# ImIntheMiddle/EmLoco

Measured on AMD Instinct MI355X. Metric: env-steps/sec (SMPL humanoid, num_envs), higher is better.
Workload: dtype f32

## Files before the change

### emloco_amd/csrc/emloco_types.h

```cpp
#pragma once
#define EMLOCO_PART_WORDS 800
#include "../../include/emloco_sim.h"
#define EMLOCO_PART_TAG(seq, part) ((seq) * 4u + (unsigned)(part))
#define EMLOCO_ERR_PART_TIMEOUT 1u

#define EMLOCO_TOPO_PARENT 0
#define EMLOCO_TOPO_DEPTH 24
#define EMLOCO_TOPO_CHILD 48
#define EMLOCO_TOPO_PDPACK 120
#define EMLOCO_TOPO_CAND 144
#define EMLOCO_TOPO_SCPAIR 240
#define EMLOCO_TOPO_WORDS 560

#define EMLOCO_MB_DYN 0
#define EMLOCO_MB_GEO 384
#define EMLOCO_MB_CAP 576
#define EMLOCO_MB_DRV 832
#define EMLOCO_MODEL_WORDS 1112

struct EmlocoSimDev {
    int n_env, n_cand, max_depth, sc_n;
    int sc_nseg;
    const int *topo;
    const float *model;
// ... 1 lines not shown
    const float *pd_target;
    float *rb_state, *contact_force, *dof_force, *lambda_ws;
    float sc_k, sc_c, sc_max_pen, sc_mu;
    const short *hf;
    int hf_nx, hf_ny;
    float hf_hs, hf_inv_hs, hf_vs, hf_ox, hf_oy, hf_pad_;
    const unsigned char *hf_mv;
    long long *prof;
    const long long *step_skip;
    const int *step_ids;
    int n_slots;
    const int *step_order;
    unsigned *step_ticks;
    int n_parts; unsigned part_seq;
    float *part_state;
    unsigned *part_flag;
    unsigned *err;
    int part_spin_max;
    int part_poison;
    unsigned long long *step_start;
    const unsigned *plan;
    int plan_n;
};
```

### emloco_amd/csrc/sim_capi.hip

```cpp
#include <hip/hip_runtime.h>
#include <cstdlib>
#include <cstdio>
#include <cstring>
#include <string>
#include <vector>
#ifdef EMLOCO_SIM_PAIR
#include "sim_pair_kernels.hip"
#define EMLOCO_SIM_ENVS_PER_WG 2
#else
#include "sim_kernels.hip"
#define EMLOCO_SIM_ENVS_PER_WG 1
#endif
#include "topology.h"
#include "model_pack.h"
#include "sim_state.h"
#include "sim_plan.h"
#include "capi_error.h"

using emloco::capi_fail;

namespace {

int check_device_error(EmlocoSim *s, const char *where) {
    if (!s->h_err) return EMLOCO_OK;
// ... 24 lines not shown

int emloco_sim_create(const EmlocoSimParams *params, int device, EmlocoSim **out) {
    if (!params || !out) return capi_fail(EMLOCO_E_ARG, "emloco_sim_create: null argument");
    if (params->n_sub < 1 || params->h <= 0.0f || params->n_iter < 0 || params->drive_mode < 0 || params->drive_mode > 1)
        return capi_fail(EMLOCO_E_ARG, "emloco_sim_create: n_sub >= 1, h > 0, n_iter >= 0, drive_mode 0 | 1 required");
    int n = 0;
    if (hipGetDeviceCount(&n) != hipSuccess || n == 0) return capi_fail(EMLOCO_E_NODEV, "no HIP device visible");
    if (device < 0 || device >= n) return capi_fail(EMLOCO_E_ARG, "emloco_sim_create: device index out of range");
    EMLOCO_HIPCHK(hipSetDevice(device));
    EmlocoSim *s = new EmlocoSim();
    s->device = device;
    s->prm = *params;
    *out = s;
    return EMLOCO_OK;
}

int emloco_sim_destroy(EmlocoSim *s) {
    if (!s) return EMLOCO_OK;
    (void)hipSetDevice(s->device);
    s->d_topo.release(); s->d_model.release();
    s->d_root.release(); s->d_dof.release(); s->d_tgt.release(); s->d_rb.release();
    s->d_cf.release(); s->d_df.release(); s->d_lws.release();
    s->d_ticks.release(); s->d_order.release(); s->d_order_ws.release();
    s->d_part_state.release(); s->d_part_flag.release(); s->d_plan.release();
    if (s->h_err) (void)hipHostFree(s->h_err);
    for (auto e : s->ev0) (void)hipEventDestroy(e);
    for (auto e : s->ev1) (void)hipEventDestroy(e);
    delete s;
    return EMLOCO_OK;
}

int emloco_sim_set_models(EmlocoSim *s, const EmlocoModelDesc *m) {
    if (!s || !m) return capi_fail(EMLOCO_E_ARG, "emloco_sim_set_models: null argument");
    if (s->prepared) return capi_fail(EMLOCO_E_STATE, "emloco_sim_set_models: sim already prepared");
    if (m->n_env < 1) return capi_fail(EMLOCO_E_ARG, "emloco_sim_set_models: n_env < 1");
    if (!s->topo.build(m->parent, m->geom_type))
        return capi_fail(EMLOCO_E_ARG, "emloco_sim_set_models: body tree must be depth-first, depth <= 8, <= 3 children, <= 96 contact candidates");
    const size_t E = (size_t)m->n_env, NBs = EMLOCO_NB, ND = EMLOCO_NDOF;
    s->n_env = m->n_env;
    s->h_off.assign(m->joint_off, m->joint_off + E * NBs * 3);
    s->h_mass.assign(m->mass, m->mass + E * NBs);
    s->h_com.assign(m->com, m->com + E * NBs * 3);
    s->h_inertia.assign(m->inertia, m->inertia + E * NBs * 6);
    s->h_ga.assign(m->geom_a, m->geom_a + E * NBs * 3);
    s->h_gb.assign(m->geom_b, m->geom_b + E * NBs * 3);
    s->h_gr.assign(m->geom_r, m->geom_r + E * NBs);
    s->h_kp.assign(m->kp, m->kp + E * ND);
// ... 159 lines not shown
int emloco_sim_tensor(EmlocoSim *s, int kind, void **dev_ptr, int64_t shape[2]) {
    if (!s || !dev_ptr || !shape) return capi_fail(EMLOCO_E_ARG, "emloco_sim_tensor: null argument");
    if (!s->prepared) return capi_fail(EMLOCO_E_STATE, "emloco_sim_tensor: call emloco_sim_prepare first");
    const int64_t E = s->n_env;
    switch (kind) {
        case EMLOCO_T_ROOT_STATE: *dev_ptr = s->d_root.p; shape[0] = E; shape[1] = 13; break;
        case EMLOCO_T_DOF_STATE: *dev_ptr = s->d_dof.p; shape[0] = E * EMLOCO_NDOF; shape[1] = 2; break;
        case EMLOCO_T_RIGID_BODY: *dev_ptr = s->d_rb.p; shape[0] = E * EMLOCO_NB; shape[1] = 13; break;
        case EMLOCO_T_CONTACT_FORCE: *dev_ptr = s->d_cf.p; shape[0] = E * EMLOCO_NB; shape[1] = 3; break;
        case EMLOCO_T_DOF_FORCE: *dev_ptr = s->d_df.p; shape[0] = E * EMLOCO_NDOF; shape[1] = 1; break;
        case EMLOCO_T_PD_TARGET: *dev_ptr = s->d_tgt.p; shape[0] = E; shape[1] = EMLOCO_NDOF; break;
        case EMLOCO_T_WARM_START: *dev_ptr = s->d_lws.p; shape[0] = E; shape[1] = EMLOCO_MAXCAND * 3; break;
        default: return capi_fail(EMLOCO_E_ARG, "emloco_sim_tensor: unknown tensor kind");
    }
    return EMLOCO_OK;
}

int emloco_sim_set_pd_targets(EmlocoSim *s, const float *dev_targets, void *stream) {
    if (!s || !dev_targets) return capi_fail(EMLOCO_E_ARG, "emloco_sim_set_pd_targets: null argument");
    if (!s->prepared) return capi_fail(EMLOCO_E_STATE, "emloco_sim_set_pd_targets: sim not prepared");
    if (dev_targets != s->d_tgt.p)
        EMLOCO_HIPCHK(hipMemcpyAsync(s->d_tgt.p, dev_targets, (size_t)s->n_env * EMLOCO_NDOF * 4, hipMemcpyDeviceToDevice, (hipStream_t)stream));
    s->prm.drive_mode = 0;
    return EMLOCO_OK;
}

int emloco_sim_set_dof_actuation_force(EmlocoSim *s, const float *dev_forces, void *stream) {
    if (!s || !dev_forces) return capi_fail(EMLOCO_E_ARG, "emloco_sim_set_dof_actuation_force: null argument");
    if (!s->prepared) return capi_fail(EMLOCO_E_STATE, "emloco_sim_set_dof_actuation_force: sim not prepared");
    if (dev_forces != s->d_tgt.p)
        EMLOCO_HIPCHK(hipMemcpyAsync(s->d_tgt.p, dev_forces, (size_t)s->n_env * EMLOCO_NDOF * 4, hipMemcpyDeviceToDevice, (hipStream_t)stream));
    s->prm.drive_mode = 1;
    return EMLOCO_OK;
}

static int launch_order(EmlocoSim *s, hipStream_t st) {
    if (s->order_ready) { s->order_ready = false; return EMLOCO_OK; }
    hipLaunchKernelGGL(emloco::sim_order_kernel, dim3(1), dim3(1024), 0, st, s->d_ticks.p, s->n_env, s->d_order.p, s->d_order_ws.p);
    EMLOCO_HIPCHK(hipGetLastError());
    return EMLOCO_OK;
}

static bool use_plan(const EmlocoSim *s, int n_sub) { return s->plan_n > 0 && s->plan_n_sub == n_sub; }

static int launch_step(EmlocoSim *s, int n_calls, EmlocoSimDev d, int n_slots, bool list, hipStream_t st) {
    EmlocoSimParams p = s->prm;
    p.n_sub = s->prm.n_sub * n_calls;
    const int slot = s->ev_head;
    const bool timed = s->timing && !list && (s->launch_no++ % s->timing_stride) == 0;
    if (timed) EMLOCO_HIPCHK(hipEventRecord(s->ev0[slot], st));
    d.n_parts = list ? 1 : (s->n_parts < p.n_sub ? s->n_parts : p.n_sub);
    d.part_seq = ++s->part_seq; d.part_state = s->d_part_state.p; d.part_flag = s->d_part_flag.p;
    d.part_spin_max = s->part_spin_max; d.part_poison = s->part_poison;
    d.n_slots = n_slots;
    unsigned grid = (unsigned)(((n_slots + EMLOCO_SIM_ENVS_PER_WG - 1) / EMLOCO_SIM_ENVS_PER_WG) * d.n_parts);
    if (!list && use_plan(s, p.n_sub)) { d.plan = s->d_plan.p; d.plan_n = s->plan_n; grid = (unsigned)s->plan_n; }
    if (d.hf) hipLaunchKernelGGL(emloco::sim_step_kernel<1>, dim3(grid), dim3(64), (size_t)s->lds_pad, st, p, d);
    else hipLaunchKernelGGL(emloco::sim_step_kernel<0>, dim3(grid), dim3(64), (size_t)s->lds_pad, st, p, d);
    EMLOCO_HIPCHK(hipGetLastError());
    if (timed) {
        EMLOCO_HIPCHK(hipEventRecord(s->ev1[slot], st));
        s->ev_head = (slot + 1) % EmlocoSim::kRing;
        if (s->ev_count < EmlocoSim::kRing) ++s->ev_count;
    }
    return EMLOCO_OK;
}

int emloco_sim_step(EmlocoSim *s, int n_calls, void *stream) {
    if (!s) return capi_fail(EMLOCO_E_ARG, "emloco_sim_step: null sim");
    if (!s->prepared) return capi_fail(EMLOCO_E_STATE, "emloco_sim_step: sim not prepared");
    if (n_calls < 1) return capi_fail(EMLOCO_E_ARG, "emloco_sim_step: n_calls < 1");
    if (const int rc = check_device_error(s, "emloco_sim_step")) return rc;
    hipStream_t st = (hipStream_t)stream;
    EmlocoSimDev d = s->dev;
    if (s->cost_order) {
        const int rc = launch_order(s, st);
        if (rc != EMLOCO_OK) return rc;
        d.step_order = s->d_order.p;
        d.step_ticks = s->d_ticks.p;
    }
    return launch_step(s, n_calls, d, s->n_env, false, st);
}

int emloco_sim_step_subset(EmlocoSim *s, int n_calls, const int64_t *dev_skip, const int32_t *dev_ids, int n_ids, void *stream) {
    if (!s) return capi_fail(EMLOCO_E_ARG, "emloco_sim_step_subset: null sim");
    if (!s->prepared) return capi_fail(EMLOCO_E_STATE, "emloco_sim_step_subset: sim not prepared");
    if (n_calls < 1) return capi_fail(EMLOCO_E_ARG, "emloco_sim_step_subset: n_calls < 1");
    if ((dev_skip == nullptr) == (dev_ids == nullptr)) return capi_fail(EMLOCO_E_ARG, "emloco_sim_step_subset: exactly one of skip flags / id list");
    if (dev_ids && (n_ids < 0 || n_ids > s->n_env)) return capi_fail(EMLOCO_E_ARG, "emloco_sim_step_subset: bad id count");
    if (dev_ids && n_ids == 0) return EMLOCO_OK;
    if (const int rc = check_device_error(s, "emloco_sim_step_subset")) return rc;
    EmlocoSimDev d = s->dev;
    d.step_skip = (const long long *)dev_skip;
    d.step_ids = (const int *)dev_ids;
    hipStream_t st = (hipStream_t)stream;
    if (s->cost_order) {
        d.step_ticks = s->d_ticks.p;
        if (dev_skip) {
            const int rc = launch_order(s, st);
            if (rc != EMLOCO_OK) return rc;
            d.step_order = s->d_order.p;
        }
    }
    return launch_step(s, n_calls, d, dev_ids ? n_ids : s->n_env, dev_ids != nullptr, st);
}

int emloco_sim_set_split(EmlocoSim *s, int n_parts) {
    if (!s) return capi_fail(EMLOCO_E_ARG, "emloco_sim_set_split: null sim");
    if (!s->prepared) return capi_fail(EMLOCO_E_STATE, "emloco_sim_set_split: sim not prepared");
    if (n_parts < 1 || n_parts > 4) return capi_fail(EMLOCO_E_ARG, "emloco_sim_set_split: 1 to 4 parts");
    if (n_parts > 1 && !s->d_part_state.p) {
        EMLOCO_HIPCHK(hipSetDevice(s->device));
// ... 176 lines not shown
```

### emloco_amd/csrc/sim_kernels.hip

```cpp
#include <hip/hip_runtime.h>
#include "dev_math.h"
#include "sim_math.h"
#define cross3 fcross3
#define dot3 fdot3
#define dot6 fdot6
#define qmul fqmul
#define qnormalize fqnormalize
#define q2mat fq2mat
#define matvec3 fmatvec3
#define rotvec2quat frotvec2quat
#define quat2rotvec fquat2rotvec
#include "emloco_types.h"
#include "fk_device.h"
#include "order_device.h"
#include "sim_plan.h"

namespace emloco {

#define NB EMLOCO_NB
#define NDOF EMLOCO_NDOF
#define MAXC EMLOCO_MAXC
#define MAXR (3 * EMLOCO_MAXC)
#define MAXCAND EMLOCO_MAXCAND
#define EMLOCO_WH_MAX 1.0f
#define YLEN 30

__device__ __forceinline__ constexpr int sidx(int a, int b) {
    return a <= b ? (a * (13 - a)) / 2 + (b - a) : (b * (13 - b)) / 2 + (a - b);
}

__device__ __forceinline__ int tri_index(int a, int b) {
    const int hi = a > b ? a : b, lo = a > b ? b : a;
    return ((hi * (hi + 1)) >> 1) + lo;
}

struct ContactMatrixSquare { static constexpr bool square = true; };
struct ContactMatrixPacked { static constexpr bool square = false; };
template <bool SQ>
// ... 187 lines not shown
                const float dv[3] = {0.0f - q[0], 0.0f - q[1], 0.0f - q[2]};
                const float side = dot3f(dv, fn);
                const float ifn = 1.0f / sqrtf(fn2);
                if (dsel >= 0.0f) {
                    const float dist = sqrtf(dot3f(dv, dv));
                    if (side >= 0.0f && dist < dsel) {
                        dsel = dist;
                        if (dist > 1.0e-6f) { const float id_ = 1.0f / dist; for (int k = 0; k < 3; ++k) nsel[k] = dv[k] * id_; }
                        else for (int k = 0; k < 3; ++k) nsel[k] = fn[k] * ifn;
                    }
                } else if (side < 0.0f && face) {
                    const float dw = side * ifn;
                    if (dw > dsel) { dsel = dw; for (int k = 0; k < 3; ++k) nsel[k] = fn[k] * ifn; }
                }
            }
        }
    }
}

#ifndef EMLOCO_SIM_WAVES_PER_SIMD
#define EMLOCO_SIM_WAVES_PER_SIMD 3
#endif
template <int HF>
__device__ __forceinline__ void sim_step_env(const EmlocoSimParams &prm, const EmlocoSimDev &d, const int env, int &work, const SimPlanWork &pw) {
    int lane = threadIdx.x;
    work = 0;

    enum { O_ROOT = 0, O_P = 16, O_V0 = 24, O_L = 36, O_PD = 48, O_R = O_PD + NB, O_W = O_R + NB * 12,
           O_L0 = O_W + NB * 24, O_CB = O_L0 + 44, O_CX = O_CB + MAXC / 4 + 3, O_CDIST = O_CX + 3 * MAXC, O_LAM = O_CDIST + MAXC,
           O_SLOT = O_LAM + MAXR, O_CRANGE = O_SLOT + 32, O_IA = O_CRANGE + 2 * NB / 4, O_G = O_IA + 180,
           O_PA = O_IA + NB * 24, O_A_ = O_PA + NB * 8, O_V = O_A_ + NB * 8,
           O_VF = O_V + NB * 8, O_AACC = O_VF + NB * 8, O_FEXT = O_AACC + NB * 8, O_PQ = O_FEXT + NB * 8,
           LDS_WORDS = (O_PQ + NB * 8 > O_G + MAXR * (MAXR + 1) / 2) ? O_PQ + NB * 8 : O_G + MAXR * (MAXR + 1) / 2 };
    static_assert(O_R % 4 == 0 && O_W % 4 == 0 && O_IA % 4 == 0 && O_PA % 4 == 0 && O_PQ % 4 == 0, "rows must be 16-byte aligned");
    static_assert(O_V - O_G >= EMLOCO_SC_MAXSEG * 8 + EMLOCO_SC_MAXHITS * 8 + 256, "limb-limb scratch does not fit its overlay");
    static_assert(LDS_WORDS * 4 <= 13312, "LDS per env above 160 KiB / 12 in 512-byte granules (three waves per SIMD, 12 envs per CU)");
    enum { SQ_MAXC = 14, SQ_ROWS = 3 * SQ_MAXC, SQ_LD = SQ_ROWS + 1 };
    static_assert(SQ_ROWS * SQ_LD <= LDS_WORDS - O_G && (SQ_ROWS - 1) * SQ_LD + SQ_ROWS + 3 <= LDS_WORDS - O_G,
                  "the square contact matrix (and the read one contact ahead of its last row) does not fit the matrix region");
    static_assert(SQ_ROWS > 32 && SQ_ROWS <= 64 && SQ_MAXC <= MAXC, "square layout: at most two tile rows of the Gram build");
    __shared__ __attribute__((aligned(16))) float lds[LDS_WORDS];
    float *sh_root = lds + O_ROOT;
    float *sh_V0 = lds + O_V0;
    float *sh_P = lds + O_P;
    float *sh_L = lds + O_L;
    int *sh_pd = (int *)(lds + O_PD);
    float (*sh_R)[12] = (float (*)[12])(lds + O_R);
// ... 13 lines not shown
    float (*sh_Vf)[8] = (float (*)[8])(lds + O_VF);
    float (*sh_Aacc)[8] = (float (*)[8])(lds + O_AACC);
    float (*sh_fext)[8] = (float (*)[8])(lds + O_FEXT);
    float (*sh_pq)[8] = (float (*)[8])(lds + O_PQ);
    float *sh_A = lds + O_G;
    constexpr bool hf_on = HF != 0;

    const int *topo = d.topo;
    const float *mdl = d.model + (size_t)env * EMLOCO_MODEL_WORDS;
#define o_dyn (EMLOCO_MB_DYN + (lane < NB ? lane : 0) * 16)
#define jdof ((lane >= 1 && lane < NB) ? (lane - 1) * 3 : 0)
#define o_drv (EMLOCO_MB_DRV + jdof * 4)
    const float *tgt_env = d.pd_target + (size_t)env * NDOF;
    float *dofs_env = d.dof_state + (size_t)env * NDOF * 2;
    float *cf_env = d.contact_force + (size_t)env * NB * 3;
    float *lws_env = d.lambda_ws + (size_t)env * MAXCAND * 3;
    const int pd_w = lane < NB ? topo[EMLOCO_TOPO_PDPACK + lane] : 0;
    float jm[4];
    ld4(mdl, o_dyn, jm);
    sh_slot[lane] = 255; sh_slot[lane + 64] = 255;

    const int part = pw.part(), sub_lo = pw.sub_lo, sub_hi = pw.sub_hi;
    float *pst = d.part_state ? d.part_state + (long)env * EMLOCO_PART_WORDS : nullptr;
    float qj[4] = {0, 0, 0, 1}, wj[3] = {0, 0, 0}, edof[3] = {0, 0, 0};
    if (!pw.consumes()) {
        if ((lane < NB) && lane >= 1) {
            const float *ds = dofs_env + jdof * 2;
            float e[3] = {ds[0], ds[2], ds[4]};
            rotvec2quat(e, qj);
            wj[0] = ds[1]; wj[1] = ds[3]; wj[2] = ds[5];
            quat2rotvec(qj, edof);
        }
        if (lane == 0) {
            const float *rs = d.root_state + (long)env * 13;
            float q0[4] = {rs[3], rs[4], rs[5], rs[6]};
            qnormalize(q0);
            for (int k = 0; k < 3; ++k) { sh_root[k] = rs[k]; sh_root[7 + k] = rs[10 + k]; sh_root[10 + k] = rs[7 + k]; }
            for (int k = 0; k < 4; ++k) sh_root[3 + k] = q0[k];
        }
    } else {
        const unsigned want = EMLOCO_PART_TAG(d.part_seq, part - 1);
        const float *pa = pst + lane * 4, *pb = lane < NB ? pst + PART_GB + lane * 4 : pa;
        float v[20];
        int spins = 0;
        bool bad;
        for (;;) {
// ... 1 lines not shown
            bool miss = __float_as_uint(v[1]) != want || __float_as_uint(v[3]) != want || __float_as_uint(v[5]) != want || __float_as_uint(v[7]) != want;
            if (lane < NB)
                for (int k = 9; k < 20; k += 2) miss = miss || __float_as_uint(v[k]) != want;
            bad = __ballot(miss) != 0ull;
            if (!bad || ++spins >= d.part_spin_max) break;
            __builtin_amdgcn_s_sleep(16);
        }
        if (bad) {
            if (lane == 0) part_err_raise(d.err, EMLOCO_ERR_PART_TIMEOUT);
            work = -1;
            return;
        }
        if ((lane < NB)) {
            qj[0] = v[0]; qj[1] = v[2]; qj[2] = v[4]; qj[3] = v[6];
            wj[0] = v[8]; wj[1] = v[10]; wj[2] = v[12];
            edof[0] = v[14]; edof[1] = v[16]; edof[2] = v[18];
        } else if (lane < NB + 32) {
            const int g = lane - NB;
            float *dst = g < 4 ? sh_root + 4 * g : g < 6 ? sh_P + 4 * (g - 4) : g < 22 ? sh_lam + 4 * (g - 6) : g < 30 ? (float *)sh_slot + 4 * (g - 22) : sh_L;
            if (g != 30) { dst[0] = v[0]; dst[1] = v[2]; dst[2] = v[4]; dst[3] = v[6]; }
        }
        work = __shfl(__float_as_int(v[0]), NB + 30);
    }
    if (lane < NB) sh_pd[lane] = pd_w;
    __syncthreads();
    SCHED_HANDED();

    const float h = prm.h;
    float tau[3], dd[3];
    int sat[3];
    float uh[3], qdd[3];

    for (int sub = sub_lo; sub < sub_hi + (pw.final() ? 1 : 0); ++sub) {
        const bool final_pass = (sub == prm.n_sub);
        const bool last = (sub == prm.n_sub - 1);

        PSTAMP(0);
        if (lane == 0) {
            float q0[4] = {sh_root[3], sh_root[4], sh_root[5], sh_root[6]}, R[9];
            q2mat(q0, R);
            for (int k = 0; k < 3; ++k) { sh_pq[0][k] = sh_root[k]; sh_R[0][9 + k] = 0.0f; }
            for (int k = 0; k < 4; ++k) sh_pq[0][4 + k] = q0[k];
            for (int k = 0; k < 9; ++k) sh_R[0][k] = R[k];
            for (int k = 0; k < 6; ++k) { sh_V[0][k] = sh_root[7 + k]; sh_Aacc[0][k] = 0.0f; }
        }
        const float joff[3] = {jm[0], jm[1], jm[2]};
// ... 1070 lines not shown
            float *ds = dofs_env + jdof * 2;
            for (int k = 0; k < 3; ++k) { ds[2 * k] = edof[k]; ds[2 * k + 1] = wj[k]; }
        }
    }
    if (lane == 0) {
        float *rs = d.root_state + (long)env * 13;
        for (int k = 0; k < 3; ++k) { rs[k] = sh_root[k]; rs[7 + k] = sh_root[10 + k]; rs[10 + k] = sh_root[7 + k]; }
        for (int k = 0; k < 4; ++k) rs[3 + k] = sh_root[3 + k];
    }
    for (int s = 0; s < 2; ++s) {
        const int c = lane + 64 * s;
        if (c < MAXCAND) {
            const int os = sh_slot[c];
            for (int k = 0; k < 3; ++k) lws_env[c * 3 + k] = os != 255 ? sh_lam[3 * os + k] : 0.0f;
        }
    }
}
#undef o_dyn
#undef jdof
#undef o_drv

template <int HF>
__global__ void __attribute__((amdgpu_flat_work_group_size(64, 64), amdgpu_waves_per_eu(EMLOCO_SIM_WAVES_PER_SIMD, EMLOCO_SIM_WAVES_PER_SIMD)))
sim_step_kernel(EmlocoSimParams prm, EmlocoSimDev d) {
    const int n_parts = d.n_parts > 1 ? d.n_parts : 1;
    const SimPlanWork pw = sim_plan_decode(d.plan, d.plan_n, blockIdx.x, d.n_env, n_parts, prm.n_sub);
    const int part = pw.part(), slot = pw.slot;
    if (!pw.valid) return;
    int env = d.step_order ? d.step_order[slot] : slot;
    if (d.step_ids) { env = d.step_ids[slot]; if (env < 0) return; }
    if (d.step_skip && d.step_skip[env] != 0) return;
    env = __builtin_amdgcn_readfirstlane(env);
    const long long t0 = d.step_start ? (long long)wall_clock64() : 0ll;
    int work;
    sim_step_env<HF>(prm, d, env, work, pw);
    if (d.step_ticks && threadIdx.x == 0 && pw.final()) {
#ifdef EMLOCO_COST_KEY_TICKS
        d.step_ticks[env] = (unsigned)(((long long)wall_clock64() - t0) >> 9);
#else
        d.step_ticks[env] = (unsigned)work;
#endif
#ifndef EMLOCO_SIM_SCHED
        if (d.step_start) { d.step_start[env] = (unsigned long long)t0; d.step_start[d.n_env + env] = (unsigned long long)wall_clock64(); }
#endif
    }
#ifdef EMLOCO_SIM_SCHED
    if (d.step_start && threadIdx.x == 0) {
        unsigned long long *ss = d.step_start + ((size_t)part * d.n_env + env) * 4;
        ss[0] = (unsigned long long)t0; ss[2] = (unsigned long long)wall_clock64(); ss[3] = (unsigned long long)(part | slot << 8) | (unsigned long long)blockIdx.x << 32;
    }
#endif
}

__global__ void __launch_bounds__(1024)
sim_order_kernel(const unsigned *ticks, int n, int *order, unsigned char *bucket_ws) {
    order_sort(ticks, n, order, bucket_ws);
}

// ... 34 lines not shown
```

### emloco_amd/csrc/sim_state.h

```cpp
#pragma once
#include <hip/hip_runtime.h>
#include <vector>
#include "emloco_types.h"
#include "topology.h"

template <class T> struct DevBuf {
    T *p = nullptr; size_t n = 0;
    hipError_t alloc(size_t count) { n = count; return hipMalloc((void **)&p, count * sizeof(T)); }
    hipError_t upload(const T *src, size_t count) {
        hipError_t e = alloc(count);
        if (e != hipSuccess) return e;
        return hipMemcpy(p, src, count * sizeof(T), hipMemcpyHostToDevice);
    }
    void release() { if (p) (void)hipFree(p); p = nullptr; n = 0; }
};

inline unsigned list_grid(int n) { return (unsigned)(n < 256 ? n : 256); }

struct EmlocoSim {
    int device = 0;
    EmlocoSimParams prm{};
    bool have_model = false, prepared = false, timing = false;
    int n_env = 0;
    emloco::Topology topo;
    std::vector<float> h_off, h_mass, h_com, h_inertia, h_ga, h_gb, h_gr, h_kp, h_kd, h_arm, h_eff;
    std::vector<unsigned char> h_sc_pairs, h_sc_segbody;
    int sc_nseg = EMLOCO_NB;
    std::vector<float> h_sc_a, h_sc_b, h_sc_r;
    float sc_k = 0.0f, sc_c = 0.0f, sc_max_pen = 0.0f, sc_mu = 0.0f;
    std::vector<short> h_hf;
    std::vector<uint8_t> h_hf_mv;
    int hf_nx = 0, hf_ny = 0;
    float hf_hs = 0.0f, hf_vs = 0.0f, hf_ox = 0.0f, hf_oy = 0.0f;
    DevBuf<short> d_hf;
    DevBuf<unsigned char> d_hf_mv;
    DevBuf<int> d_topo;
    DevBuf<float> d_model;
    DevBuf<float> d_root, d_dof, d_tgt, d_rb, d_cf, d_df, d_lws;
    EmlocoSimDev dev{};
    int n_parts = 1;
    unsigned part_seq = 0;
    DevBuf<float> d_part_state;
    DevBuf<unsigned> d_part_flag;
    unsigned *h_err = nullptr;
    int part_spin_max = 1 << 22, part_poison = -1;
    DevBuf<unsigned> d_plan;
    int plan_n = 0, plan_n_sub = 0;
    int lds_pad = 0;
    bool cost_order = false;
    bool order_ready = false;
    DevBuf<unsigned> d_ticks;
    DevBuf<int> d_order;
    DevBuf<unsigned char> d_order_ws;
    static constexpr int kRing = 1024;
    std::vector<hipEvent_t> ev0, ev1;
    int ev_head = 0, ev_count = 0;
    int timing_stride = 1, launch_no = 0;
    float last_ms = -1.0f;
};
```

### emloco_amd/env/tasks/humanoid.py

```python
import numpy as np
import torch

from ... import _lib as L
from ...gym import gymapi, gymtorch
from ...gym.torch_utils import get_axis_params, to_torch
from ...model import smpl_humanoid
from ...post_physics import BODY_NAMES, LEFT_TO_RIGHT, PostPhysics, dof_subset_indices
from ...utils.flags import flags
from .base_task import BaseTask

ENABLE_MAX_COORD_OBS = True


class Humanoid(BaseTask):
    def __init__(self, cfg, sim_params, physics_engine, device_type, device_id, headless):
        self.cfg = cfg
        self.sim_params = sim_params
        self.physics_engine = physics_engine
        self.has_task = getattr(self, "has_task", False)
        self.device_type, self.device_id = device_type, device_id
        self.device = "cpu"
        if device_type == "cuda" or device_type == "GPU":
            self.device = "cuda" + ":" + str(device_id)
        self.load_smpl_configs(cfg)
        self._pd_control = self.cfg["env"]["pdControl"]
        self.power_scale = self.cfg["env"]["powerScale"]
        self.plane_static_friction = self.cfg["env"]["plane"]["staticFriction"]
        self.plane_dynamic_friction = self.cfg["env"]["plane"]["dynamicFriction"]
        self.plane_restitution = self.cfg["env"]["plane"]["restitution"]
# ... 302 lines not shown
        return

    def _refresh_sim_tensors(self):
        self.gym.refresh_dof_state_tensor(self.sim)
        self.gym.refresh_actor_root_state_tensor(self.sim)
        self.gym.refresh_rigid_body_state_tensor(self.sim)
        self.gym.refresh_force_sensor_tensor(self.sim)
        self.gym.refresh_dof_force_tensor(self.sim)
        self.gym.refresh_net_contact_force_tensor(self.sim)
        return

    def pre_physics_step(self, actions):
        self.wait_obs()
        if getattr(self, "_actions_buf", None) is None or self._actions_buf.shape != actions.shape:
            self._actions_buf = torch.empty(actions.shape, dtype=torch.float32, device=self.device)
        if not self._pd_control:
            self._actions_buf.copy_(actions)
            self.actions = self._actions_buf
            forces = self.actions * self.motor_efforts.unsqueeze(0) * self.power_scale
            if not self.gym.set_dof_actuation_force_tensor(self.sim, gymtorch.unwrap_tensor(forces.contiguous())):
                raise RuntimeError("set_dof_actuation_force_tensor failed (simulator not prepared, or a tensor of the wrong shape / dtype)")
            return
        src = actions.to(device=self.device, dtype=torch.float32).contiguous()
        self._post.pd_targets(src, self._pd_action_offset, self._pd_action_scale, self._pd_zero_mask, self._pd_targets,
                              actions_copy=self._actions_buf)
        self.actions = self._actions_buf
        if not self.gym.set_dof_position_target_tensor(self.sim, gymtorch.unwrap_tensor(self._pd_targets)):
            raise RuntimeError("set_dof_position_target_tensor failed (simulator not prepared, or a tensor of the wrong shape / dtype)")
        return

    def _action_to_pd_targets(self, action):
        return self._pd_action_offset + self._pd_action_scale * action

    def _post_mode_step(self):
        return L.POST_ADVANCE | L.POST_OBS | L.POST_REWARD | L.POST_RESET

    _returns_hook = None
    _returns_in_flags = False

    def attach_returns(self, step_struct, before=None):
        self._returns_hook = step_struct
        self._returns_before = before if step_struct is not None else None

    def _launch_post(self, mode, env_ids=None):
        if self._post_bufs is None:
            self._post_bufs = self._make_post_bufs()
            if hasattr(self, "_amp_ring_to_bufs"):
                self._amp_ring_to_bufs()
        if (self._returns_hook is not None and env_ids is None and (mode & L.POST_REWARD) and (mode & L.POST_RESET)
                and not (mode & L.POST_SKIP_DONE)):
            if getattr(self, "_returns_before", None) is not None:
                self._returns_before()
# ... 74 lines not shown
```

### emloco_amd/sim.py

```python
import ctypes as C

import numpy as np
import torch

from . import _lib as L
from .model import HumanoidModel, pack_models

_TORCH_TYPESTR = {torch.float32: "<f4", torch.int32: "<i4", torch.int64: "<i8", torch.uint8: "|u1", torch.int16: "<i2"}


class _DevView:

    def __init__(self, ptr, shape, dtype, owner):
        self.__cuda_array_interface__ = {"shape": tuple(int(s) for s in shape), "typestr": _TORCH_TYPESTR[dtype],
                                         "data": (int(ptr), False), "version": 2, "strides": None}
        self._owner = owner


def wrap_device_pointer(ptr, shape, dtype, device, owner=None):
    return torch.as_tensor(_DevView(ptr, shape, dtype, owner), device=device)


def current_stream_handle(device):
    return C.c_void_p(torch.cuda.current_stream(device).cuda_stream)
# ... 9 lines not shown

def plan_from_spec(spec, n_env, n_sub, parts=4):
    spec = (spec or "").strip()
    if spec in ("", "0"):
        return None
    parts = min(parts, n_sub)
    tail, shift, k, light_parts = False, 0, 0, parts
    for term in spec.split("+"):
        term = term.strip()
        if term == "T":
            tail = True
            continue
        if not term or term[0] not in "CS":
            raise L.EmlocoError(f"part plan {spec!r}: unknown term {term!r}")
        body, _, sh = term[1:].partition(":")
        k = int(round(n_env * float(body[:-1]) / 100.0)) if body.endswith("%") else int(body)
        k = max(0, min(n_env, k))
        if term[0] == "C":
            light_parts = max(1, parts // 2)
        else:
            shift = int(sh or 1)
    classes = [(0, n_env - k, parts), (n_env - k, n_env, light_parts)] if k else [(0, n_env, parts)]
    return classes, tail, shift


class NativeSim:
    def __init__(self, models, params=None, device_index=0, self_collision=None, heightfield=None):
        lib = L.require_device()
        self.lib = lib
        self.device_index = int(device_index)
        self.device = torch.device("cuda", self.device_index)
        self.params = params or L.default_sim_params()
        if isinstance(models, dict):
            packed = models
        else:
            if isinstance(models, HumanoidModel):
                models = [models]
            packed = pack_models(models)
        self._packed = {k: np.ascontiguousarray(v) for k, v in packed.items()}
        self.num_envs = int(self._packed["mass"].shape[0])
        self._h = C.c_void_p()
        L.check(lib.emloco_sim_create(C.byref(self.params), self.device_index, C.byref(self._h)), "emloco_sim_create")
        p = self._packed
        f = lambda a: a.ctypes.data_as(C.POINTER(C.c_float))
        i = lambda a: a.ctypes.data_as(C.POINTER(C.c_int32))
        desc = L.ModelDesc(self.num_envs, i(p["parent"]), i(p["geom_type"]), f(p["joint_off"]), f(p["mass"]),
# ... 16 lines not shown
            hf = np.ascontiguousarray(heightfield["samples"], dtype=np.int16)
            if hf.ndim != 2:
                raise L.EmlocoError("heightfield samples must be a 2-D int16 array [nx][ny]")
            L.check(lib.emloco_sim_set_ground_heightfield(
                self._h, hf.ctypes.data, hf.shape[0], hf.shape[1], float(heightfield["horizontal_scale"]),
                float(heightfield["vertical_scale"]), float(heightfield.get("origin_x", 0.0)),
                float(heightfield.get("origin_y", 0.0))), "emloco_sim_set_ground_heightfield")
            if heightfield.get("move_x") is not None:
                mx = np.ascontiguousarray(heightfield["move_x"], dtype=np.int8)
                my = np.ascontiguousarray(heightfield["move_y"], dtype=np.int8)
                if mx.shape != hf.shape or my.shape != hf.shape:
                    raise L.EmlocoError("heightfield move_x / move_y must have the samples' shape")
                L.check(lib.emloco_sim_set_ground_mesh_moves(self._h, mx.ctypes.data, my.ctypes.data), "emloco_sim_set_ground_mesh_moves")
        L.check(lib.emloco_sim_prepare(self._h), "emloco_sim_prepare")
        self.root_state = self._tensor(L.T_ROOT_STATE)
        self.dof_state = self._tensor(L.T_DOF_STATE)
        self.rigid_body_state = self._tensor(L.T_RIGID_BODY)
        self.contact_force = self._tensor(L.T_CONTACT_FORCE)
        self.dof_force = self._tensor(L.T_DOF_FORCE).view(-1)
        self.pd_target = self._tensor(L.T_PD_TARGET)
        self.warm_start = self._tensor(L.T_WARM_START)
        self._plan_spec, self._plan_parts, self._plan_calls = None, 4, 0
        self.drive_mode = int(self.params.drive_mode)

    def _tensor(self, kind):
        ptr = C.c_void_p()
        shape = (C.c_int64 * 2)()
        L.check(self.lib.emloco_sim_tensor(self._h, kind, C.byref(ptr), shape), "emloco_sim_tensor")
        return wrap_device_pointer(ptr.value, (shape[0], shape[1]), torch.float32, self.device, owner=self)

    def _stream(self):
        return current_stream_handle(self.device)

    def set_pd_targets(self, targets):
        L.check(self.lib.emloco_sim_set_pd_targets(self._h, dptr(targets), self._stream()), "emloco_sim_set_pd_targets")
        self.drive_mode = 0

    def set_dof_actuation_force(self, forces):
        if forces.dtype != torch.float32 or forces.numel() != self.num_envs * 69:
            raise L.EmlocoError("actuation forces must be a float32 [n_env][69] tensor")
        L.check(self.lib.emloco_sim_set_dof_actuation_force(self._h, dptr(forces), self._stream()), "emloco_sim_set_dof_actuation_force")
        self.drive_mode = 1

    def step(self, n_calls=1):
        if self._plan_spec is not None and self._plan_calls != n_calls:
            self._plan_for(n_calls)
        L.check(self.lib.emloco_sim_step(self._h, int(n_calls), self._stream()), "emloco_sim_step")

    def set_cost_order(self, on=True):
        L.check(self.lib.emloco_sim_set_cost_order(self._h, int(bool(on))), "emloco_sim_set_cost_order")

    def set_split(self, n_parts=2):
        L.check(self.lib.emloco_sim_set_split(self._h, int(n_parts)), "emloco_sim_set_split")
        self._plan_spec = None

    def set_plan(self, classes, tail=False, shift=0, n_calls=1):
        flat = np.ascontiguousarray(np.asarray(classes, dtype=np.int32).reshape(-1, 3))
        L.check(self.lib.emloco_sim_set_plan(self._h, flat.ctypes.data_as(C.POINTER(C.c_int32)), int(flat.shape[0]), int(bool(tail)), int(shift),
                                             int(n_calls)), "emloco_sim_set_plan")
        self._plan_spec = None

    def set_plan_spec(self, spec, parts=4):
        self._plan_spec, self._plan_parts, self._plan_calls = (spec if plan_from_spec(spec, self.num_envs, 4) is not None else None), parts, 0

    def _plan_for(self, n_calls):
        plan = plan_from_spec(self._plan_spec, self.num_envs, int(self.get_params().n_sub) * n_calls, self._plan_parts)
        spec = self._plan_spec
        try:
            self.set_plan(*plan, n_calls=n_calls)
        except L.EmlocoError:
# ... 62 lines not shown
```

### include/emloco_sim.h

```cpp
#ifndef EMLOCO_SIM_H
#define EMLOCO_SIM_H
#include <stdint.h>

#ifdef __cplusplus
extern "C" {
#endif

#define EMLOCO_NB 24
#define EMLOCO_NDOF 69
#define EMLOCO_MAXC 20
#define EMLOCO_MAXCAND 96

enum { EMLOCO_GEOM_SPHERE = 0, EMLOCO_GEOM_CAPSULE = 1, EMLOCO_GEOM_BOX = 2 };

enum {
    EMLOCO_OK = 0,
    EMLOCO_E_ARG = -1,
    EMLOCO_E_HIP = -2,
    EMLOCO_E_STATE = -3,
    EMLOCO_E_NODEV = -4
};

typedef struct {
    int32_t n_sub;
// ... 52 lines not shown
    EMLOCO_T_PD_TARGET = 5,
    EMLOCO_T_WARM_START = 6,
    EMLOCO_T_COUNT = 7
};

typedef struct EmlocoSim EmlocoSim;

const char *emloco_last_error(void);
int emloco_device_count(void);

int emloco_sim_create(const EmlocoSimParams *params, int device, EmlocoSim **out);
int emloco_sim_destroy(EmlocoSim *sim);
int emloco_sim_set_models(EmlocoSim *sim, const EmlocoModelDesc *desc);
int emloco_sim_set_self_collision(EmlocoSim *sim, const EmlocoSelfCollisionDesc *desc);
int emloco_sim_set_ground_heightfield(EmlocoSim *sim, const int16_t *samples, int nx, int ny, float horizontal_scale,
                                      float vertical_scale, float origin_x, float origin_y);
int emloco_sim_set_ground_mesh_moves(EmlocoSim *sim, const int8_t *move_x, const int8_t *move_y);
int emloco_sim_prepare(EmlocoSim *sim);
int emloco_sim_get_params(EmlocoSim *sim, EmlocoSimParams *out);
int emloco_sim_set_params(EmlocoSim *sim, const EmlocoSimParams *in);
int emloco_sim_tensor(EmlocoSim *sim, int kind, void **dev_ptr, int64_t shape[2]);
int emloco_sim_set_pd_targets(EmlocoSim *sim, const float *dev_targets, void *stream);
int emloco_sim_set_dof_actuation_force(EmlocoSim *sim, const float *dev_forces, void *stream);
int emloco_sim_step(EmlocoSim *sim, int n_calls, void *stream);
int emloco_sim_step_subset(EmlocoSim *sim, int n_calls, const int64_t *dev_skip, const int32_t *dev_env_ids, int n_ids, void *stream);
int emloco_sim_set_split(EmlocoSim *sim, int n_parts);
int emloco_sim_set_plan(EmlocoSim *sim, const int32_t *classes, int n_classes, int tail, int shift, int n_calls);
int emloco_sim_set_cost_order(EmlocoSim *sim, int on);
int emloco_sim_sync(EmlocoSim *sim, void *stream);
int emloco_sim_debug_poison_part(EmlocoSim *sim, int env, int spin_max);
int emloco_sim_fk_indexed(EmlocoSim *sim, const int32_t *dev_env_ids, int n, void *stream);
int emloco_sim_cost_ticks(EmlocoSim *sim, unsigned *host_ticks, unsigned long long *host_start, int n);
int emloco_sim_profile(EmlocoSim *sim, long long *host_out, int n);
int emloco_sim_set_root_state_indexed(EmlocoSim *sim, const float *dev_full, const int32_t *dev_env_ids, int n, void *stream);
int emloco_sim_set_dof_state_indexed(EmlocoSim *sim, const float *dev_full, const int32_t *dev_env_ids, int n, void *stream);
int emloco_sim_refresh_bodies(EmlocoSim *sim, void *stream);
int emloco_sim_num_candidates(EmlocoSim *sim);
float emloco_sim_last_step_ms(EmlocoSim *sim);
int emloco_sim_enable_timing(EmlocoSim *sim, int on);
int emloco_sim_timing_stats(EmlocoSim *sim, int *n_launches, float *total_ms);

#ifdef __cplusplus
}
#endif
#endif
```

Before: 10.03 million.

## Fuse action-to-PD-target mapping into the simulation step kernel

Adds a path where raw policy actions and a per-DOF (offset, scale, zero-mask) map are handed to the step kernel, which computes PD targets per lane in-kernel instead of a separate post-processing kernel plus a target-tensor set. For split-part plans, consuming parts write targets into a new staging buffer so the shared target tensor is not raced, and the first part also writes the actions copy. This removes one or more small launches and a global round trip per env step. In exchange it adds loads and some register pressure in the hot kernel, and it is enabled by default through an environment flag.

```diff
diff --git a/emloco_amd/csrc/emloco_types.h b/emloco_amd/csrc/emloco_types.h
--- a/emloco_amd/csrc/emloco_types.h
+++ b/emloco_amd/csrc/emloco_types.h
@@ -47,3 +47,10 @@
     const unsigned *plan;
     int plan_n;
 };
+
+struct EmlocoSimAct {
+    const float *act;
+    const float *map;
+    float *copy;
+    float *stage;
+};
diff --git a/emloco_amd/csrc/sim_act_device.h b/emloco_amd/csrc/sim_act_device.h
--- /dev/null
+++ b/emloco_amd/csrc/sim_act_device.h
@@ -0,0 +1,38 @@
+#pragma once
+#include "emloco_types.h"
+
+namespace emloco {
+
+__device__ __forceinline__ float act_form(const float *rec, float a) { return rec[2] != 0.0f ? 0.0f : rec[0] + rec[1] * a; }
+
+__device__ __forceinline__ void act_ld4(const float *p, float *v) {
+#ifdef EMLOCO_EMU
+    for (int k = 0; k < 4; ++k) v[k] = p[k];
+#else
+    typedef float f4 __attribute__((ext_vector_type(4)));
+    const f4 r = *(const f4 *)p;
+    v[0] = r.x; v[1] = r.y; v[2] = r.z; v[3] = r.w;
+#endif
+}
+
+__device__ __forceinline__ bool act_wanted(const EmlocoSimAct &ac, int sub_lo, int sub_hi) { return ac.act != nullptr && sub_hi > sub_lo; }
+
+__device__ __forceinline__ void act_request(const EmlocoSimAct &ac, bool on, int env, int lane, int jd, float a[3], float rec[3][4]) {
+    for (int k = 0; k < 3; ++k) { a[k] = 0.0f; rec[k][0] = rec[k][1] = rec[k][2] = rec[k][3] = 0.0f; }
+    if (on && lane >= 1 && lane < EMLOCO_NB)
+        for (int k = 0; k < 3; ++k) { act_ld4(ac.map + (jd + k) * 4, rec[k]); a[k] = ac.act[(size_t)env * EMLOCO_NDOF + jd + k]; }
+}
+
+__device__ __forceinline__ const float *act_fill(const EmlocoSimAct &ac, bool on, bool consumes, int part, int n_env, int env, int lane, int jd,
+                                                 const float a[3], const float rec[3][4], const float *tgt_env) {
+    if (!on) return tgt_env;
+    float *row = consumes ? ac.stage + ((size_t)(part - 1) * n_env + env) * EMLOCO_NDOF : const_cast<float *>(tgt_env);
+    if (lane >= 1 && lane < EMLOCO_NB)
+        for (int k = 0; k < 3; ++k) {
+            row[jd + k] = act_form(rec[k], a[k]);
+            if (!consumes && ac.copy) ac.copy[(size_t)env * EMLOCO_NDOF + jd + k] = a[k];
+        }
+    return row;
+}
+
+}
diff --git a/emloco_amd/csrc/sim_capi.hip b/emloco_amd/csrc/sim_capi.hip
--- a/emloco_amd/csrc/sim_capi.hip
+++ b/emloco_amd/csrc/sim_capi.hip
@@ -70,7 +70,7 @@
     s->d_root.release(); s->d_dof.release(); s->d_tgt.release(); s->d_rb.release();
     s->d_cf.release(); s->d_df.release(); s->d_lws.release();
     s->d_ticks.release(); s->d_order.release(); s->d_order_ws.release();
-    s->d_part_state.release(); s->d_part_flag.release(); s->d_plan.release();
+    s->d_part_state.release(); s->d_part_flag.release(); s->d_plan.release(); s->d_act_stage.release();
     if (s->h_err) (void)hipHostFree(s->h_err);
     for (auto e : s->ev0) (void)hipEventDestroy(e);
     for (auto e : s->ev1) (void)hipEventDestroy(e);
@@ -276,6 +276,21 @@
     if (dev_targets != s->d_tgt.p)
         EMLOCO_HIPCHK(hipMemcpyAsync(s->d_tgt.p, dev_targets, (size_t)s->n_env * EMLOCO_NDOF * 4, hipMemcpyDeviceToDevice, (hipStream_t)stream));
     s->prm.drive_mode = 0;
+    s->act = EmlocoSimAct{nullptr, nullptr, nullptr, nullptr};
+    return EMLOCO_OK;
+}
+
+int emloco_sim_set_action_targets(EmlocoSim *s, const float *dev_actions, const float *dev_action_map, float *dev_actions_copy) {
+    if (!s || !dev_actions || !dev_action_map) return capi_fail(EMLOCO_E_ARG, "emloco_sim_set_action_targets: null argument");
+    if (!s->prepared) return capi_fail(EMLOCO_E_STATE, "emloco_sim_set_action_targets: sim not prepared");
+    if (EMLOCO_SIM_ENVS_PER_WG != 1) return capi_fail(EMLOCO_E_ARG, "emloco_sim_set_action_targets: one env per workgroup only");
+    if (dev_actions == s->d_tgt.p) return capi_fail(EMLOCO_E_ARG, "emloco_sim_set_action_targets: the actions must not be the sim's own target tensor");
+    if (!s->d_act_stage.p) {
+        EMLOCO_HIPCHK(hipSetDevice(s->device));
+        EMLOCO_HIPCHK(s->d_act_stage.alloc((size_t)(EMLOCO_PLAN_MAX_PARTS - 1) * (size_t)s->n_env * EMLOCO_NDOF));
+    }
+    s->act = EmlocoSimAct{dev_actions, dev_action_map, dev_actions_copy != dev_actions ? dev_actions_copy : nullptr, s->d_act_stage.p};
+    s->prm.drive_mode = 0;
     return EMLOCO_OK;
 }
 
@@ -285,6 +300,7 @@
     if (dev_forces != s->d_tgt.p)
         EMLOCO_HIPCHK(hipMemcpyAsync(s->d_tgt.p, dev_forces, (size_t)s->n_env * EMLOCO_NDOF * 4, hipMemcpyDeviceToDevice, (hipStream_t)stream));
     s->prm.drive_mode = 1;
+    s->act = EmlocoSimAct{nullptr, nullptr, nullptr, nullptr};
     return EMLOCO_OK;
 }
 
@@ -297,7 +313,8 @@
 
 static bool use_plan(const EmlocoSim *s, int n_sub) { return s->plan_n > 0 && s->plan_n_sub == n_sub; }
 
-static int launch_step(EmlocoSim *s, int n_calls, EmlocoSimDev d, int n_slots, bool list, hipStream_t st) {
+static int launch_step(EmlocoSim *s, int n_calls, EmlocoSimDev d, int n_slots, bool list, hipStream_t st,
+                       EmlocoSimAct ac = EmlocoSimAct{nullptr, nullptr, nullptr, nullptr}) {
     EmlocoSimParams p = s->prm;
     p.n_sub = s->prm.n_sub * n_calls;
     const int slot = s->ev_head;
@@ -309,8 +326,13 @@
     d.n_slots = n_slots;
     unsigned grid = (unsigned)(((n_slots + EMLOCO_SIM_ENVS_PER_WG - 1) / EMLOCO_SIM_ENVS_PER_WG) * d.n_parts);
     if (!list && use_plan(s, p.n_sub)) { d.plan = s->d_plan.p; d.plan_n = s->plan_n; grid = (unsigned)s->plan_n; }
+#if EMLOCO_SIM_ENVS_PER_WG == 1
+    if (d.hf) hipLaunchKernelGGL(emloco::sim_step_kernel<1>, dim3(grid), dim3(64), (size_t)s->lds_pad, st, p, d, ac);
+    else hipLaunchKernelGGL(emloco::sim_step_kernel<0>, dim3(grid), dim3(64), (size_t)s->lds_pad, st, p, d, ac);
+#else
     if (d.hf) hipLaunchKernelGGL(emloco::sim_step_kernel<1>, dim3(grid), dim3(64), (size_t)s->lds_pad, st, p, d);
     else hipLaunchKernelGGL(emloco::sim_step_kernel<0>, dim3(grid), dim3(64), (size_t)s->lds_pad, st, p, d);
+#endif
     EMLOCO_HIPCHK(hipGetLastError());
     if (timed) {
         EMLOCO_HIPCHK(hipEventRecord(s->ev1[slot], st));
@@ -333,7 +355,9 @@
         d.step_order = s->d_order.p;
         d.step_ticks = s->d_ticks.p;
     }
-    return launch_step(s, n_calls, d, s->n_env, false, st);
+    const EmlocoSimAct ac = s->act;
+    s->act = EmlocoSimAct{nullptr, nullptr, nullptr, nullptr};
+    return launch_step(s, n_calls, d, s->n_env, false, st, ac);
 }
 
 int emloco_sim_step_subset(EmlocoSim *s, int n_calls, const int64_t *dev_skip, const int32_t *dev_ids, int n_ids, void *stream) {
@@ -342,6 +366,7 @@
     if (n_calls < 1) return capi_fail(EMLOCO_E_ARG, "emloco_sim_step_subset: n_calls < 1");
     if ((dev_skip == nullptr) == (dev_ids == nullptr)) return capi_fail(EMLOCO_E_ARG, "emloco_sim_step_subset: exactly one of skip flags / id list");
     if (dev_ids && (n_ids < 0 || n_ids > s->n_env)) return capi_fail(EMLOCO_E_ARG, "emloco_sim_step_subset: bad id count");
+    if (s->act.act) return capi_fail(EMLOCO_E_STATE, "emloco_sim_step_subset: an action source is armed (emloco_sim_set_action_targets); a subset launch takes emloco_sim_set_pd_targets");
     if (dev_ids && n_ids == 0) return EMLOCO_OK;
     if (const int rc = check_device_error(s, "emloco_sim_step_subset")) return rc;
     EmlocoSimDev d = s->dev;
diff --git a/emloco_amd/csrc/sim_kernels.hip b/emloco_amd/csrc/sim_kernels.hip
--- a/emloco_amd/csrc/sim_kernels.hip
+++ b/emloco_amd/csrc/sim_kernels.hip
@@ -14,6 +14,7 @@
 #include "fk_device.h"
 #include "order_device.h"
 #include "sim_plan.h"
+#include "sim_act_device.h"
 
 namespace emloco {
 
@@ -247,7 +248,7 @@
 #define EMLOCO_SIM_WAVES_PER_SIMD 3
 #endif
 template <int HF>
-__device__ __forceinline__ void sim_step_env(const EmlocoSimParams &prm, const EmlocoSimDev &d, const int env, int &work, const SimPlanWork &pw) {
+__device__ __forceinline__ void sim_step_env(const EmlocoSimParams &prm, const EmlocoSimDev &d, const EmlocoSimAct &ac, const int env, int &work, const SimPlanWork &pw) {
     int lane = threadIdx.x;
     work = 0;
 
@@ -307,6 +308,9 @@
 
     const int part = pw.part(), sub_lo = pw.sub_lo, sub_hi = pw.sub_hi;
     float *pst = d.part_state ? d.part_state + (long)env * EMLOCO_PART_WORDS : nullptr;
+    const bool act_on = act_wanted(ac, sub_lo, sub_hi);
+    float act_a[3], act_rec[3][4];
+    act_request(ac, act_on, env, lane, jdof, act_a, act_rec);
     float qj[4] = {0, 0, 0, 1}, wj[3] = {0, 0, 0}, edof[3] = {0, 0, 0};
     if (!pw.consumes()) {
         if ((lane < NB) && lane >= 1) {
@@ -354,6 +358,7 @@
         }
         work = __shfl(__float_as_int(v[0]), NB + 30);
     }
+    tgt_env = act_fill(ac, act_on, pw.consumes(), part, d.n_env, env, lane, jdof, act_a, act_rec, tgt_env);
     if (lane < NB) sh_pd[lane] = pd_w;
     __syncthreads();
     SCHED_HANDED();
@@ -1470,7 +1475,7 @@
 
 template <int HF>
 __global__ void __attribute__((amdgpu_flat_work_group_size(64, 64), amdgpu_waves_per_eu(EMLOCO_SIM_WAVES_PER_SIMD, EMLOCO_SIM_WAVES_PER_SIMD)))
-sim_step_kernel(EmlocoSimParams prm, EmlocoSimDev d) {
+sim_step_kernel(EmlocoSimParams prm, EmlocoSimDev d, EmlocoSimAct ac = EmlocoSimAct{nullptr, nullptr, nullptr, nullptr}) {
     const int n_parts = d.n_parts > 1 ? d.n_parts : 1;
     const SimPlanWork pw = sim_plan_decode(d.plan, d.plan_n, blockIdx.x, d.n_env, n_parts, prm.n_sub);
     const int part = pw.part(), slot = pw.slot;
@@ -1481,7 +1486,7 @@
     env = __builtin_amdgcn_readfirstlane(env);
     const long long t0 = d.step_start ? (long long)wall_clock64() : 0ll;
     int work;
-    sim_step_env<HF>(prm, d, env, work, pw);
+    sim_step_env<HF>(prm, d, ac, env, work, pw);
     if (d.step_ticks && threadIdx.x == 0 && pw.final()) {
 #ifdef EMLOCO_COST_KEY_TICKS
         d.step_ticks[env] = (unsigned)(((long long)wall_clock64() - t0) >> 9);
diff --git a/emloco_amd/csrc/sim_state.h b/emloco_amd/csrc/sim_state.h
--- a/emloco_amd/csrc/sim_state.h
+++ b/emloco_amd/csrc/sim_state.h
@@ -38,6 +38,8 @@
     DevBuf<float> d_model;
     DevBuf<float> d_root, d_dof, d_tgt, d_rb, d_cf, d_df, d_lws;
     EmlocoSimDev dev{};
+    DevBuf<float> d_act_stage;
+    EmlocoSimAct act{};
     int n_parts = 1;
     unsigned part_seq = 0;
     DevBuf<float> d_part_state;
diff --git a/emloco_amd/env/tasks/humanoid.py b/emloco_amd/env/tasks/humanoid.py
--- a/emloco_amd/env/tasks/humanoid.py
+++ b/emloco_amd/env/tasks/humanoid.py
@@ -1,3 +1,5 @@
+import os
+
 import numpy as np
 import torch
 
@@ -5,6 +7,7 @@
 from ...gym import gymapi, gymtorch
 from ...gym.torch_utils import get_axis_params, to_torch
 from ...model import smpl_humanoid
+from ...sim import action_target_map
 from ...post_physics import BODY_NAMES, LEFT_TO_RIGHT, PostPhysics, dof_subset_indices
 from ...utils.flags import flags
 from .base_task import BaseTask
@@ -353,12 +356,32 @@
                 raise RuntimeError("set_dof_actuation_force_tensor failed (simulator not prepared, or a tensor of the wrong shape / dtype)")
             return
         src = actions.to(device=self.device, dtype=torch.float32).contiguous()
+        if self._fuse_pd_targets(src):
+            self.sim.native.set_action_targets(src, self._action_target_map(), self._actions_buf)
+            self.actions = self._actions_buf
+            return
         self._post.pd_targets(src, self._pd_action_offset, self._pd_action_scale, self._pd_zero_mask, self._pd_targets,
                               actions_copy=self._actions_buf)
         self.actions = self._actions_buf
         if not self.gym.set_dof_position_target_tensor(self.sim, gymtorch.unwrap_tensor(self._pd_targets)):
             raise RuntimeError("set_dof_position_target_tensor failed (simulator not prepared, or a tensor of the wrong shape / dtype)")
         return
+
+    fused_pd_targets = os.environ.get("EMLOCO_FUSED_PD_TARGETS", "1") != "0"
+
+    def _fuse_pd_targets(self, src):
+        native = getattr(self.sim, "native", None)
+        return (self.fused_pd_targets and native is not None and hasattr(native, "set_action_targets")
+                and src.shape == (self.num_envs, self.num_dof) and self._pd_targets.data_ptr() == native.pd_target.data_ptr()
+                and not getattr(self, "_rs_pending", False) and getattr(self, "before_physics_launch", None) is None
+                and not self.paused and self.enable_viewer_sync)
+
+    def _action_target_map(self):
+        key = tuple((id(t), t._version) for t in (self._pd_action_offset, self._pd_action_scale, self._pd_zero_mask))
+        if getattr(self, "_pd_map_key", None) != key:
+            self._pd_map = action_target_map(self._pd_action_offset, self._pd_action_scale, self._pd_zero_mask)
+            self._pd_map_key = key
+        return self._pd_map
 
     def _action_to_pd_targets(self, action):
         return self._pd_action_offset + self._pd_action_scale * action
diff --git a/emloco_amd/sim.py b/emloco_amd/sim.py
--- a/emloco_amd/sim.py
+++ b/emloco_amd/sim.py
@@ -55,6 +55,14 @@
             shift = int(sh or 1)
     classes = [(0, n_env - k, parts), (n_env - k, n_env, light_parts)] if k else [(0, n_env, parts)]
     return classes, tail, shift
+
+
+def action_target_map(offset, scale, zero_mask):
+    m = torch.zeros((offset.numel(), 4), dtype=torch.float32, device=offset.device)
+    m[:, 0] = offset.to(torch.float32)
+    m[:, 1] = scale.to(torch.float32)
+    m[:, 2] = (zero_mask != 0).to(torch.float32)
+    return m
 
 
 class NativeSim:
@@ -117,6 +125,7 @@
         self.warm_start = self._tensor(L.T_WARM_START)
         self._plan_spec, self._plan_parts, self._plan_calls = None, 4, 0
         self.drive_mode = int(self.params.drive_mode)
+        self._armed = None
 
     def _tensor(self, kind):
         ptr = C.c_void_p()
@@ -131,6 +140,18 @@
         L.check(self.lib.emloco_sim_set_pd_targets(self._h, dptr(targets), self._stream()), "emloco_sim_set_pd_targets")
         self.drive_mode = 0
 
+    def set_action_targets(self, actions, action_map, actions_copy=None):
+        if actions.dtype != torch.float32 or not actions.is_contiguous() or actions.numel() != self.num_envs * 69:
+            raise L.EmlocoError("actions must be a contiguous float32 [n_env][69] tensor")
+        if action_map.dtype != torch.float32 or not action_map.is_contiguous() or action_map.numel() != 69 * 4:
+            raise L.EmlocoError("the action map must be a contiguous float32 [69][4] tensor")
+        if actions_copy is not None and (actions_copy.dtype != torch.float32 or not actions_copy.is_contiguous() or actions_copy.numel() != actions.numel()):
+            raise L.EmlocoError("the actions copy must be a contiguous float32 [n_env][69] tensor")
+        L.check(self.lib.emloco_sim_set_action_targets(self._h, dptr(actions), dptr(action_map), dptr(actions_copy)),
+                "emloco_sim_set_action_targets")
+        self._armed = (actions, action_map, actions_copy)
+        self.drive_mode = 0
+
     def set_dof_actuation_force(self, forces):
         if forces.dtype != torch.float32 or forces.numel() != self.num_envs * 69:
             raise L.EmlocoError("actuation forces must be a float32 [n_env][69] tensor")
@@ -141,6 +162,7 @@
         if self._plan_spec is not None and self._plan_calls != n_calls:
             self._plan_for(n_calls)
         L.check(self.lib.emloco_sim_step(self._h, int(n_calls), self._stream()), "emloco_sim_step")
+        self._armed = None
 
     def set_cost_order(self, on=True):
         L.check(self.lib.emloco_sim_set_cost_order(self._h, int(bool(on))), "emloco_sim_set_cost_order")
diff --git a/include/emloco_sim.h b/include/emloco_sim.h
--- a/include/emloco_sim.h
+++ b/include/emloco_sim.h
@@ -98,6 +98,7 @@
 int emloco_sim_tensor(EmlocoSim *sim, int kind, void **dev_ptr, int64_t shape[2]);
 int emloco_sim_set_pd_targets(EmlocoSim *sim, const float *dev_targets, void *stream);
 int emloco_sim_set_dof_actuation_force(EmlocoSim *sim, const float *dev_forces, void *stream);
+int emloco_sim_set_action_targets(EmlocoSim *sim, const float *dev_actions, const float *dev_action_map, float *dev_actions_copy);
 int emloco_sim_step(EmlocoSim *sim, int n_calls, void *stream);
 int emloco_sim_step_subset(EmlocoSim *sim, int n_calls, const int64_t *dev_skip, const int32_t *dev_env_ids, int n_ids, void *stream);
 int emloco_sim_set_split(EmlocoSim *sim, int n_parts);
```

Measured after the change: 10.03 million (median of 5 runs). No clear change (+0.1%).
